# deepomicslab/PALACE

Measured on AMD Instinct MI355X. Metric: contigs/sec eref+generate_graph+matching, 1M-contig synth, 1/2/4/8 GPU, higher is better.
Workload: dtype u32

## Files before the change

palace_amd/csrc/decomp.hip:

```cpp
#include "decomp.hpp"

#include <algorithm>

namespace palace {

namespace {

constexpr uint64_t kNoKey = ~0ull;
constexpr uint64_t kClosed = 0;
constexpr int kStampShift = 42;
constexpr int kPackedShift = 52, kPackedStamps = 1 << (64 - kPackedShift);
constexpr uint64_t kLenMask = (1ull << 40) - 1;


__device__ __forceinline__ uint64_t wave_incl_scan(uint64_t v, int lane)
{
#pragma unroll
    for (int d = 1; d < 64; d <<= 1) {
        const uint64_t u = __shfl_up(v, d);
        if (lane >= d) v += u;
    }
    return v;
}

constexpr int kMaxWaves = 16;

__device__ void scan_partials_body(const uint64_t *__restrict__ in, int64_t n, uint64_t *__restrict__ partials, int blk, int nblk)
{
    __shared__ uint64_t part[kMaxWaves];
    const int64_t chunk = (n + nblk - 1) / nblk;
    const int64_t a = min(n, static_cast<int64_t>(blk) * chunk), e = min(n, a + chunk);
    uint64_t s = 0;
    for (int64_t i = a + threadIdx.x; i < e; i += blockDim.x) s += in[i];
    const int lane = threadIdx.x & 63, waves = static_cast<int>(blockDim.x >> 6);
    s = wave_incl_scan(s, lane);
    if (lane == 63) part[threadIdx.x >> 6] = s;
    __syncthreads();
    if (threadIdx.x == 0) {
        uint64_t t = 0;
        for (int w = 0; w < waves; w++) t += part[w];
        partials[blk] = t;
    }
    __syncthreads();
}

__device__ void scan_prefix_body(uint64_t *__restrict__ partials, int n_parts, uint64_t *__restrict__ total)
{
    __shared__ uint64_t part[kMaxWaves];
    const int lane = threadIdx.x & 63, wv = threadIdx.x >> 6;
    const uint64_t x = static_cast<int>(threadIdx.x) < n_parts ? partials[threadIdx.x] : 0;
    const uint64_t incl = wave_incl_scan(x, lane);
    if (lane == 63) part[wv] = incl;
    __syncthreads();
    uint64_t before = 0;
    for (int w = 0; w < wv; w++) before += part[w];
    if (static_cast<int>(threadIdx.x) < n_parts) partials[threadIdx.x] = before + incl - x;
    if (threadIdx.x == blockDim.x - 1) *total = before + incl;
    __syncthreads();
}

__device__ void scan_apply_body(const uint64_t *__restrict__ in, uint64_t *__restrict__ out, int64_t n, const uint64_t *__restrict__ partials,
                                int blk, int nblk)
{
    __shared__ uint64_t part[kMaxWaves];
    const int64_t chunk = (n + nblk - 1) / nblk;
    const int64_t a = min(n, static_cast<int64_t>(blk) * chunk), e = min(n, a + chunk);
    const int lane = threadIdx.x & 63, wv = threadIdx.x >> 6, waves = static_cast<int>(blockDim.x >> 6);
    uint64_t carry = partials[blk];
    for (int64_t base = a; base < e; base += blockDim.x) {
        const int64_t i = base + threadIdx.x;
        const uint64_t x = i < e ? in[i] : 0;
        const uint64_t incl = wave_incl_scan(x, lane);
        if (lane == 63) part[wv] = incl;
        __syncthreads();
        uint64_t before = 0, all = 0;
        for (int w = 0; w < waves; w++) { if (w < wv) before += part[w]; all += part[w]; }
        if (i < e) out[i] = carry + before + incl - x;
        carry += all;
        __syncthreads();
    }
}

__global__ __launch_bounds__(kDecompBlock) void scan_partials_kernel(const uint64_t *__restrict__ in, const int32_t *__restrict__ n_dev,
                                                                     uint64_t *__restrict__ partials)
{
    scan_partials_body(in, *n_dev, partials, static_cast<int>(blockIdx.x), static_cast<int>(gridDim.x));
}
__global__ __launch_bounds__(kDecompBlock) void scan_prefix_kernel(uint64_t *__restrict__ partials, int n_parts, uint64_t *__restrict__ total)
{
    scan_prefix_body(partials, n_parts, total);
}
__global__ __launch_bounds__(kDecompBlock) void scan_apply_kernel(const uint64_t *__restrict__ in, uint64_t *__restrict__ out,
                                                                  const int32_t *__restrict__ n_dev, const uint64_t *__restrict__ partials)
{
    scan_apply_body(in, out, *n_dev, partials, static_cast<int>(blockIdx.x), static_cast<int>(gridDim.x));
}

struct Span { int tid, n; };
__device__ __forceinline__ Span whole_grid() { return Span{static_cast<int>(blockIdx.x * blockDim.x + threadIdx.x), static_cast<int>(gridDim.x * blockDim.x)}; }

__device__ void ph_init(const DecompBufs &b, Span T, int64_t comp_cap, int64_t vert_cap, int n_flags, int allow_packed)
{
    DecompState *st = b.st;
    const int V = st->V;
    for (int i = T.tid; i < V; i += T.n) { b.bo_hi[i] = kNoKey; b.bi_hi[i] = kNoKey; b.on_path[i] = 0; }
    for (int i = T.tid; i < n_flags; i += T.n) b.changed[i] = 0;
    if (T.tid == 0) {
        st->n_comp = 0; st->n_vert = 0; st->comp_cap = comp_cap; st->vert_cap = vert_cap;
        st->unsettled = 0; st->overflow = 0; st->bad = 0; st->dead = 0; st->scan_total = 0; st->alive_after = 0;
        st->packed = (allow_packed && b.kc && b.pack_bad && *b.pack_bad == 0) ? 1u : 0u;
        if (comp_cap >= 0) b.o_off[0] = 0;
    }
}

__device__ void ph_round_begin(const DecompBufs &b, Span T, int reset_left)
{
    const int V = b.st->V;
    if (!reset_left && b.st->dead) return;
    if (T.tid == 0) { b.st->alive_after = 0; if (reset_left) b.st->dead = 0; }
    const int64_t E = b.st->E;
    for (int64_t e = T.tid; e < E; e += T.n) b.done[e] = 0;
    const bool packed = b.st->packed != 0;
    for (int i = T.tid; i < V; i += T.n) {
        const int s = i >> 1;
        const int64_t l = reset_left ? 1 : b.left[s];
        if (reset_left && !(i & 1)) b.left[s] = 1;
        b.alive[i] = l > 0;
        b.next[i] = -1; b.prev[i] = -1;
        b.bo_hi[i] = b.bi_hi[i] = l > 0 ? kNoKey : kClosed;
        if (!packed) { b.bo_lo[i] = kNoKey; b.bo_lo[V + i] = kNoKey; b.bi_lo[i] = kNoKey; b.bi_lo[V + i] = kNoKey; }
        b.len_a[i] = 0;
    }
}

struct IterArgs {
    uint64_t stamp;
    uint64_t stamp_p;
    int parity;
    int prev_flag, flag;
    int unique_hi;
};


__device__ void ph_propose_hi(const DecompBufs &b, Span T, const IterArgs &a)
{
    if (b.st->dead) return;
    if (a.prev_flag >= 0 && !b.changed[a.prev_flag]) return;
    const int64_t E = b.st->E;
    const int V = b.st->V;
    const int other = (a.parity ^ 1) * V;
    const bool packed = b.st->packed != 0;
    for (int64_t e = T.tid; e < E; e += T.n) {
        if (b.done[e]) continue;
        const int u = b.src[e], v = b.dst[e];
        if (b.bi_hi[v] == kClosed) { b.done[e] = 1; continue; }
        const uint64_t k = packed ? (a.stamp_p | b.kc[e]) : (a.stamp | b.khi[e]);
        if (atomicMin(reinterpret_cast<unsigned long long *>(&b.bo_hi[u]), static_cast<unsigned long long>(k)) == kClosed) { b.done[e] = 1; continue; }
        atomicMin(reinterpret_cast<unsigned long long *>(&b.bi_hi[v]), static_cast<unsigned long long>(k));
        if (!a.unique_hi && !packed) { b.bo_lo[other + u] = kNoKey; b.bi_lo[other + v] = kNoKey; }
    }
}

__device__ void ph_propose_lo(const DecompBufs &b, Span T, const IterArgs &a)
{
    if (b.st->dead) return;
    if (a.prev_flag >= 0 && !b.changed[a.prev_flag]) return;
    if (b.st->packed) return;
    const int64_t E = b.st->E;
    const int mine = a.parity * b.st->V;
    for (int64_t e = T.tid; e < E; e += T.n) {
        if (b.done[e]) continue;
        const int u = b.src[e], v = b.dst[e];
        const uint64_t k = a.stamp | b.khi[e], lo = b.klo[e];
        if (b.bo_hi[u] == k) atomicMin(reinterpret_cast<unsigned long long *>(&b.bo_lo[mine + u]), static_cast<unsigned long long>(lo));
        if (b.bi_hi[v] == k) atomicMin(reinterpret_cast<unsigned long long *>(&b.bi_lo[mine + v]), static_cast<unsigned long long>(lo));
    }
}

__device__ void ph_commit_flag(const DecompBufs &b, Span T, const IterArgs &a, volatile unsigned int *took);
__device__ void ph_commit(const DecompBufs &b, Span T, const IterArgs &a)
{
    if (b.st->dead) return;
    if (a.prev_flag >= 0 && !b.changed[a.prev_flag]) return;
    ph_commit_flag(b, T, a, b.changed + a.flag);
}
__device__ void ph_commit_flag(const DecompBufs &b, Span T, const IterArgs &a, volatile unsigned int *took)
{
    bool any = false;
    const int64_t E = b.st->E;
    const int mine = a.parity * b.st->V;
    const bool packed = b.st->packed != 0;
    for (int64_t e = T.tid; e < E; e += T.n) {
        if (b.done[e]) continue;
        const int u = b.src[e], v = b.dst[e];
        const uint64_t k = packed ? (a.stamp_p | b.kc[e]) : (a.stamp | b.khi[e]);
        if (b.bo_hi[u] != k || b.bi_hi[v] != k) continue;
        const uint64_t lo = b.klo[e];
        if (!a.unique_hi && !packed && (b.bo_lo[mine + u] != lo || b.bi_lo[mine + v] != lo)) continue;
        b.next[u] = v; b.prev[v] = u;
        b.nhi[u] = b.khi[e]; b.nlo[u] = lo;
        b.bo_hi[u] = kClosed; b.bi_hi[v] = kClosed;
        b.done[e] = 1;
        any = true;
    }
    if (__syncthreads_or(any) && threadIdx.x == 0) *took = 1u;
}

__device__ void ph_heads(const DecompBufs &b, Span T, int round, int last_flag)
{
    DecompState *st = b.st;
    if (st->dead) return;
    if (T.tid == 0 && last_flag >= 0 && b.changed[last_flag]) st->unsettled = 1;
    const int V = st->V;
    for (int v = T.tid; v < V; v += T.n) {
        if (!b.alive[v] || b.prev[v] >= 0) continue;
        int len = 0, last = v;
        int64_t least = b.left[v >> 1];
        for (int x = v; x >= 0; x = b.next[x]) {
            b.on_path[x] = round + 1;
            last = x;
            len++;
            least = min(least, b.left[x >> 1]);
        }
        const int twin_first = last ^ 1;
        if (v > twin_first) continue;
        const int64_t uses = twin_first == v ? 2 : 1;
        b.len_a[v] = (1ull << 40) | static_cast<uint64_t>(len);
        b.pay[v] = max(static_cast<int64_t>(1), least / uses);
        b.kind[v] = 0;
        b.open_at[v] = 0;
    }
}

__device__ void ph_cycles(const DecompBufs &b, Span T, int round)
{
    const int V = b.st->V;
    if (b.st->dead) return;
    for (int v = T.tid; v < V; v += T.n) {
        if (!b.alive[v] || b.on_path[v] == round + 1) continue;
        int len = 1, twin_least = v ^ 1, worst = 0;
        uint64_t whi = b.nhi[v], wlo = b.nlo[v];
        int64_t least = b.left[v >> 1];
        bool first = true;
        for (int x = b.next[v]; x != v; x = b.next[x]) {
            if (x < v) { first = false; break; }
            twin_least = min(twin_least, x ^ 1);
            const uint64_t hi = b.nhi[x], lo = b.nlo[x];
            if (hi > whi || (hi == whi && lo > wlo)) { whi = hi; wlo = lo; worst = len; }
            least = min(least, b.left[x >> 1]);
            len++;
        }
        if (!first || v > twin_least) continue;
        const int64_t uses = twin_least == v ? 2 : 1;
        b.len_a[v] = (1ull << 40) | static_cast<uint64_t>(len);
        b.pay[v] = max(static_cast<int64_t>(1), least / uses);
        b.kind[v] = 1;
        b.open_at[v] = (worst + 1) % len;
    }
}

__device__ void ph_emit(const DecompBufs &b, Span T, int round, int64_t c0, int64_t v0)
{
    DecompState *st = b.st;
    const int V = st->V;
    if (st->dead) return;
    int64_t alive = 0;
    for (int v = T.tid; v < V; v += T.n) {
        const uint64_t la = b.len_a[v];
        if (!la) continue;
        const int64_t len = static_cast<int64_t>(la & kLenMask);
        const uint64_t p = b.pos[v];
        const int64_t c = c0 + static_cast<int64_t>(p >> 40), at = v0 + static_cast<int64_t>(p & kLenMask);
        const int64_t pay = b.pay[v];
        const bool room = c < st->comp_cap && at + len <= st->vert_cap;
        if (!room) st->overflow = 1;
        else { b.o_off[c] = at; b.o_kind[c] = b.kind[v]; b.o_iter[c] = round; b.o_open[c] = b.open_at[v]; }
        int x = v;
        int64_t still = 0;
        for (int64_t k = 0; k < len; k++) {
            if (room) b.o_verts[at + k] = 2 * b.orig[x >> 1] + (x & 1);
            const int64_t l = b.left[x >> 1];
            b.left[x >> 1] = max(static_cast<int64_t>(0), l - pay);
            still += l - pay > 0;
            x = b.next[x];
        }
        alive += still;
    }
    __shared__ unsigned long long wg_alive;
    if (threadIdx.x == 0) wg_alive = 0;
    __syncthreads();
    if (alive) atomicAdd(&wg_alive, static_cast<unsigned long long>(alive));
    __syncthreads();
    if (threadIdx.x == 0 && wg_alive) atomicAdd(reinterpret_cast<unsigned long long *>(&st->alive_after), wg_alive);
}


__global__ void dec_init_kernel(DecompBufs b, int64_t comp_cap, int64_t vert_cap, int n_flags, int allow_packed) { ph_init(b, whole_grid(), comp_cap, vert_cap, n_flags, allow_packed); }
__global__ void dec_round_begin_kernel(DecompBufs b, int reset_left) { ph_round_begin(b, whole_grid(), reset_left); }
__global__ void dec_propose_hi_kernel(DecompBufs b, IterArgs a) { ph_propose_hi(b, whole_grid(), a); }
__global__ void dec_propose_lo_kernel(DecompBufs b, IterArgs a) { ph_propose_lo(b, whole_grid(), a); }
__global__ void dec_commit_kernel(DecompBufs b, IterArgs a) { ph_commit(b, whole_grid(), a); }
__global__ void dec_heads_kernel(DecompBufs b, int round, int last_flag) { ph_heads(b, whole_grid(), round, last_flag); }
__global__ void dec_cycles_kernel(DecompBufs b, int round) { ph_cycles(b, whole_grid(), round); }
__global__ void dec_emit_kernel(DecompBufs b, int round) { ph_emit(b, whole_grid(), round, b.st->n_comp, b.st->n_vert); }

__global__ void dec_round_end_kernel(DecompBufs b)
{
    DecompState *st = b.st;
    if (blockIdx.x || threadIdx.x || st->dead) return;
    st->dead = st->alive_after == 0;
    st->n_comp += static_cast<int64_t>(st->scan_total >> 40);
    st->n_vert += static_cast<int64_t>(st->scan_total & kLenMask);
    if (st->n_comp <= st->comp_cap) b.o_off[st->n_comp] = st->n_vert;
}

size_t up256(size_t v) { return (v + 255) / 256 * 256; }

struct Carver {
    char *base;
    size_t used = 0;
    template <class T>
    T *take(size_t n)
    {
        T *p = base ? reinterpret_cast<T *>(base + used) : nullptr;
        used += up256(std::max<size_t>(1, n) * sizeof(T));
        return p;
    }
};

size_t carve_all(DecompBufs &b, char *base, int64_t s_cap, int64_t e_cap, int64_t comp_cap, int64_t vert_cap, int rounds, int iters)
{
    Carver c{base};
    const size_t S = static_cast<size_t>(std::max<int64_t>(1, s_cap)), V = 2 * S, E = static_cast<size_t>(std::max<int64_t>(1, e_cap));
    b.st = c.take<DecompState>(1);
    b.src = c.take<int32_t>(E); b.dst = c.take<int32_t>(E);
    b.khi = c.take<uint64_t>(E); b.klo = c.take<uint64_t>(E);
    b.done = c.take<uint8_t>(E);
    b.kc = c.take<uint64_t>(E);
    b.left = c.take<int64_t>(S); b.orig = c.take<int32_t>(S);
    b.next = c.take<int32_t>(V); b.prev = c.take<int32_t>(V); b.on_path = c.take<int32_t>(V); b.open_at = c.take<int32_t>(V);
    b.nhi = c.take<uint64_t>(V); b.nlo = c.take<uint64_t>(V);
    b.bo_hi = c.take<uint64_t>(V); b.bi_hi = c.take<uint64_t>(V);
    b.bo_lo = c.take<uint64_t>(2 * V); b.bi_lo = c.take<uint64_t>(2 * V);
    b.len_a = c.take<uint64_t>(V); b.pos = c.take<uint64_t>(V);
    b.pay = c.take<int64_t>(V);
    b.alive = c.take<uint8_t>(V); b.kind = c.take<uint8_t>(V);
    b.partials = c.take<uint64_t>(kDecompGrid + 1);
    b.changed = c.take<uint32_t>(static_cast<size_t>(rounds) * static_cast<size_t>(iters));
    b.o_off = c.take<int64_t>(static_cast<size_t>(comp_cap) + 1);
    b.o_verts = c.take<int32_t>(static_cast<size_t>(vert_cap));
    b.o_iter = c.take<int32_t>(static_cast<size_t>(comp_cap));
    b.o_open = c.take<int32_t>(static_cast<size_t>(comp_cap));
    b.o_kind = c.take<uint8_t>(static_cast<size_t>(comp_cap));
    return c.used;
}

}

size_t decomp_bytes(int64_t s_cap, int64_t e_cap, int64_t comp_cap, int64_t vert_cap, int rounds, int iters)
{
    DecompBufs tmp;
    return carve_all(tmp, nullptr, s_cap, e_cap, comp_cap, vert_cap, rounds, iters);
}

void decomp_carve(DecompBufs &b, char *base, int64_t s_cap, int64_t e_cap, int64_t comp_cap, int64_t vert_cap, int rounds, int iters)
{
    carve_all(b, base, s_cap, e_cap, comp_cap, vert_cap, rounds, iters);
}

int scan_u64(palace_ctx *ctx, const uint64_t *in, uint64_t *out, const int32_t *n_dev, uint64_t *partials, uint64_t *total_dev)
{
    hipLaunchKernelGGL(scan_partials_kernel, dim3(kDecompGrid), dim3(kDecompBlock), 0, ctx->stream, in, n_dev, partials);
    hipLaunchKernelGGL(scan_prefix_kernel, dim3(1), dim3(kDecompBlock), 0, ctx->stream, partials, kDecompGrid, total_dev);
    hipLaunchKernelGGL(scan_apply_kernel, dim3(kDecompGrid), dim3(kDecompBlock), 0, ctx->stream, in, out, n_dev, partials);
    PALACE_HIP_TRY(hipGetLastError());
    return PALACE_OK;
}

namespace {

const dim3 kBlock(kDecompBlock);
constexpr int kWideGridDefault = 2048;
inline dim3 wide_grid(const palace_ctx *ctx) { return dim3(ctx->match_grid > 0 ? ctx->match_grid : kWideGridDefault); }

void enqueue_iterations(palace_ctx *ctx, const DecompBufs &b, int first, int n, uint64_t *count, int flag0, bool unique_hi)
{
    for (int k = 0; k < n; k++) {
        IterArgs a{((1ull << 21) - 1 - *count) << kStampShift, static_cast<uint64_t>((kPackedStamps - 1 - *count) & (kPackedStamps - 1)) << kPackedShift,
                   (first + k) & 1, k ? flag0 + k - 1 : -1, flag0 + k, unique_hi ? 1 : 0};
        (*count)++;
        hipLaunchKernelGGL(dec_propose_hi_kernel, wide_grid(ctx), kBlock, 0, ctx->stream, b, a);
        if (!unique_hi) hipLaunchKernelGGL(dec_propose_lo_kernel, wide_grid(ctx), kBlock, 0, ctx->stream, b, a);
        hipLaunchKernelGGL(dec_commit_kernel, wide_grid(ctx), kBlock, 0, ctx->stream, b, a);
    }
}

int enqueue_read_off(palace_ctx *ctx, const DecompBufs &b, int round, int last_flag)
{
    hipLaunchKernelGGL(dec_heads_kernel, wide_grid(ctx), kBlock, 0, ctx->stream, b, round, last_flag);
    hipLaunchKernelGGL(dec_cycles_kernel, wide_grid(ctx), kBlock, 0, ctx->stream, b, round);
    int rc = scan_u64(ctx, b.len_a, b.pos, &b.st->V, b.partials, &b.st->scan_total);
    if (rc) return rc;
    hipLaunchKernelGGL(dec_emit_kernel, wide_grid(ctx), kBlock, 0, ctx->stream, b, round);
    hipLaunchKernelGGL(dec_round_end_kernel, dim3(1), dim3(64), 0, ctx->stream, b);
    PALACE_HIP_TRY(hipGetLastError());
    return PALACE_OK;
}

}

int decomp_begin(palace_ctx *ctx, const DecompBufs &b, int rounds, int64_t comp_cap, int64_t vert_cap)
{
    PALACE_REQUIRE(rounds >= 1 && rounds <= kMaxRounds, "round count out of range");
    static_assert(kDecompGrid <= kDecompBlock, "scan_prefix_kernel scans the block sums with one workgroup");
    const int allow_packed = !ctx->match_two_word_keys && static_cast<int64_t>(rounds) * kMaxIters < kPackedStamps ? 1 : 0;
    hipLaunchKernelGGL(dec_init_kernel, wide_grid(ctx), kBlock, 0, ctx->stream, b, comp_cap, vert_cap, rounds * kMaxIters, allow_packed);
    PALACE_HIP_TRY(hipGetLastError());
    return PALACE_OK;
}

int decomp_rounds(palace_ctx *ctx, const DecompBufs &b, int t0, int t1, int rounds, int aggressive, int iters, bool unique_hi,
                  uint64_t *count)
{
    PALACE_REQUIRE(0 <= t0 && t0 <= t1 && t1 <= rounds && rounds <= kMaxRounds && iters >= 1 && iters <= kMaxIters, "round / iteration count out of range");
    for (int t = t0; t < t1; t++) {
        hipLaunchKernelGGL(dec_round_begin_kernel, wide_grid(ctx), kBlock, 0, ctx->stream, b, (aggressive && t == rounds - 1) ? 1 : 0);
        enqueue_iterations(ctx, b, 0, iters, count, t * kMaxIters, unique_hi);
        int rc = enqueue_read_off(ctx, b, t, t * kMaxIters + iters - 1);
        if (rc) return rc;
    }
    PALACE_HIP_TRY(hipGetLastError());
    return PALACE_OK;
}

int decomp_run_checked(palace_ctx *ctx, const DecompBufs &b, int rounds, int aggressive, bool unique_hi, int64_t comp_cap,
                       int64_t vert_cap, int64_t max_iterations, uint64_t *iterations_out)
{
    PALACE_REQUIRE(rounds >= 1 && rounds <= kMaxRounds, "round count out of range");
    constexpr int kBatch = 16;
    hipLaunchKernelGGL(dec_init_kernel, wide_grid(ctx), kBlock, 0, ctx->stream, b, comp_cap, vert_cap, kBatch, 0);
    uint64_t count = 0;
    for (int t = 0; t < rounds; t++) {
        hipLaunchKernelGGL(dec_round_begin_kernel, wide_grid(ctx), kBlock, 0, ctx->stream, b, (aggressive && t == rounds - 1) ? 1 : 0);
        for (int first = 0;; first += kBatch) {
            PALACE_HIP_TRY(hipMemsetAsync(b.changed, 0, kBatch * sizeof(uint32_t), ctx->stream));
            enqueue_iterations(ctx, b, first, kBatch, &count, 0, unique_hi);
            uint32_t last = 0;
            PALACE_HIP_TRY(hipMemcpyAsync(&last, b.changed + kBatch - 1, sizeof last, hipMemcpyDeviceToHost, ctx->stream));
            PALACE_HIP_TRY(hipStreamSynchronize(ctx->stream));
            if (!last) break;
            if (static_cast<int64_t>(count) > max_iterations || count + kBatch >= (1ull << 21)) {
                set_error("matching: no fixed point after %llu iterations", static_cast<unsigned long long>(count));
                return PALACE_ESTATE;
            }
        }
        PALACE_HIP_TRY(hipMemsetAsync(b.changed, 0, kBatch * sizeof(uint32_t), ctx->stream));
        int rc = enqueue_read_off(ctx, b, t, kBatch - 1);
        if (rc) return rc;
    }
    if (iterations_out) *iterations_out = count;
    return PALACE_OK;
}

int decomp_group(palace_ctx *ctx, const DecompBufs &b, DecompRun &run, int rounds, int aggressive, bool unique_hi)
{
    const int first = kFirstGroupRounds;
    const int t0 = run.next_round, t1 = std::min(rounds, t0 + (t0 == 0 ? first : kRoundsPerGroup));
    for (int t = t0; t < t1; t++) {
        const int iters = ctx->match_iters > 0 ? std::min(ctx->match_iters, kMaxIters) : (t == 0 ? kFirstRoundIters : kLaterRoundIters);
        int rc = decomp_rounds(ctx, b, t, t + 1, rounds, aggressive, iters, unique_hi, &run.count);
        if (rc) return rc;
        run.rounds++;
    }
    run.next_round = t1;
    return PALACE_OK;
}

int decomp_finish(palace_ctx *ctx, const DecompBufs &b, DecompRun &run, int rounds, int aggressive, bool unique_hi, int64_t comp_cap,
                  int64_t vert_cap, int64_t max_iterations, DecompState *h_state, const std::function<int()> &reset_left)
{
    for (;;) {
        PALACE_HIP_TRY(hipMemcpyAsync(h_state, b.st, sizeof *h_state, hipMemcpyDeviceToHost, ctx->stream));
        PALACE_HIP_TRY(hipStreamSynchronize(ctx->stream));
        if (h_state->unsettled) {
            int rc = reset_left();
            if (rc) return rc;
            run.checked = true; run.rounds = rounds; run.count = 0;
            rc = decomp_run_checked(ctx, b, rounds, aggressive, unique_hi, comp_cap, vert_cap, max_iterations, &run.count);
            if (rc) return rc;
            PALACE_HIP_TRY(hipMemcpyAsync(h_state, b.st, sizeof *h_state, hipMemcpyDeviceToHost, ctx->stream));
            PALACE_HIP_TRY(hipStreamSynchronize(ctx->stream));
            return PALACE_OK;
        }
        if (run.next_round >= rounds) return PALACE_OK;
        if (h_state->alive_after == 0) {
            if (!aggressive) return PALACE_OK;
            run.next_round = rounds - 1;
        }
        int rc = decomp_group(ctx, b, run, rounds, aggressive, unique_hi);
        if (rc) return rc;
    }
}

}
```

palace_amd/csrc/decomp.hpp:

```cpp
#pragma once
#include <functional>

#include "common.hpp"

struct palace_match_result {
    int64_t n = 0;
    int64_t *off = nullptr;
    int32_t *verts = nullptr, *iter = nullptr, *open_at = nullptr;
    uint8_t *kind = nullptr;
    uint64_t *bare = nullptr;
    int64_t n_bare = 0;
    bool borrowed = false;
    ~palace_match_result();
};

namespace palace {

constexpr int kDecompGrid = 256;
constexpr int kDecompBlock = 256;
constexpr int kMaxRounds = 1024;
constexpr int kMaxIters = 64;

struct DecompState {
    int32_t S, V;
    int64_t E;
    int64_t n_comp, n_vert;
    int64_t comp_cap, vert_cap;
    uint32_t unsettled;
    uint32_t overflow;
    uint32_t bad;
    uint32_t dead;
    uint32_t packed;
    uint64_t scan_total;
    int64_t alive_after;
};

struct DecompBufs {
    DecompState *st = nullptr;
    int32_t *src = nullptr, *dst = nullptr;
    uint64_t *khi = nullptr, *klo = nullptr;
    uint8_t *done = nullptr;
    uint64_t *kc = nullptr;
    const uint32_t *pack_bad = nullptr;
    int64_t *left = nullptr;
    int32_t *orig = nullptr;
    int32_t *next = nullptr, *prev = nullptr, *on_path = nullptr, *open_at = nullptr;
    uint64_t *nhi = nullptr, *nlo = nullptr;
    uint64_t *bo_hi = nullptr, *bi_hi = nullptr;
    uint64_t *bo_lo = nullptr, *bi_lo = nullptr;
    uint64_t *len_a = nullptr, *pos = nullptr;
    int64_t *pay = nullptr;
    uint8_t *alive = nullptr, *kind = nullptr;
    uint64_t *partials = nullptr;
    uint32_t *changed = nullptr;
    int64_t *o_off = nullptr;
    int32_t *o_verts = nullptr, *o_iter = nullptr, *o_open = nullptr;
    uint8_t *o_kind = nullptr;
};

size_t decomp_bytes(int64_t s_cap, int64_t e_cap, int64_t comp_cap, int64_t vert_cap, int rounds, int iters);
void decomp_carve(DecompBufs &b, char *base, int64_t s_cap, int64_t e_cap, int64_t comp_cap, int64_t vert_cap, int rounds, int iters);
constexpr int kFirstRoundIters = 7, kLaterRoundIters = 4, kRoundsPerGroup = 5, kFirstGroupRounds = 5;
int decomp_begin(palace_ctx *ctx, const DecompBufs &b, int rounds, int64_t comp_cap, int64_t vert_cap);
int decomp_rounds(palace_ctx *ctx, const DecompBufs &b, int t0, int t1, int rounds, int aggressive, int iters, bool unique_hi,
                  uint64_t *count);

struct DecompRun { int next_round = 0; uint64_t count = 0; int rounds = 0; bool checked = false; };
int decomp_group(palace_ctx *ctx, const DecompBufs &b, DecompRun &run, int rounds, int aggressive, bool unique_hi);
int decomp_finish(palace_ctx *ctx, const DecompBufs &b, DecompRun &run, int rounds, int aggressive, bool unique_hi, int64_t comp_cap,
                  int64_t vert_cap, int64_t max_iterations, DecompState *h_state, const std::function<int()> &reset_left);

int decomp_run_checked(palace_ctx *ctx, const DecompBufs &b, int rounds, int aggressive, bool unique_hi, int64_t comp_cap,
                       int64_t vert_cap, int64_t max_iterations, uint64_t *iterations_out = nullptr);

inline void decomp_note_run(palace_ctx *ctx, const DecompRun &run, const DecompState &h_state, bool unique_hi)
{
    ctx->match_last[0] = unique_hi ? 0 : (h_state.packed ? 2 : 1);
    ctx->match_last[1] = run.checked ? 1 : 0;
    ctx->match_last[2] = run.rounds;
    ctx->match_last[3] = static_cast<int64_t>(run.count);
}

int scan_u64(palace_ctx *ctx, const uint64_t *in, uint64_t *out, const int32_t *n_dev, uint64_t *partials, uint64_t *total_dev);

}
```

Before: 112.7 million.

## Replace edge-parallel atomicMin matching with per-vertex compacted adjacency lists

Builds per-vertex out/in adjacency lists once at decomposition start (count, scan, fill) and rewrites each matching iteration as a per-slot scan that drops closed neighbours, compacts the list in place and picks the best arc, with long lists handled by a whole wave. Commit becomes vertex-parallel, checking that both endpoints chose the same arc. This removes the per-iteration pass over all edges with 64-bit atomicMin, the separate lo-key propose kernel, and the stamp bookkeeping. In exchange it adds list-building kernels, more memory for entries, and irregular per-vertex work that may be imbalanced.

```diff
diff --git a/palace_amd/csrc/decomp.hip b/palace_amd/csrc/decomp.hip
--- a/palace_amd/csrc/decomp.hip
+++ b/palace_amd/csrc/decomp.hip
@@ -6,10 +6,8 @@
 
 namespace {
 
-constexpr uint64_t kNoKey = ~0ull;
-constexpr uint64_t kClosed = 0;
-constexpr int kStampShift = 42;
-constexpr int kPackedShift = 52, kPackedStamps = 1 << (64 - kPackedShift);
+constexpr int kPackedStamps = 1 << 12;
+constexpr int kLongList = 64;
 constexpr uint64_t kLenMask = (1ull << 40) - 1;
 
 
@@ -103,13 +101,38 @@
 {
     DecompState *st = b.st;
     const int V = st->V;
-    for (int i = T.tid; i < V; i += T.n) { b.bo_hi[i] = kNoKey; b.bi_hi[i] = kNoKey; b.on_path[i] = 0; }
+    for (int i = T.tid; i < V; i += T.n) { b.cnt[i] = 0; b.cnt[V + i] = 0; b.on_path[i] = 0; }
     for (int i = T.tid; i < n_flags; i += T.n) b.changed[i] = 0;
     if (T.tid == 0) {
         st->n_comp = 0; st->n_vert = 0; st->comp_cap = comp_cap; st->vert_cap = vert_cap;
-        st->unsettled = 0; st->overflow = 0; st->bad = 0; st->dead = 0; st->scan_total = 0; st->alive_after = 0;
+        st->unsettled = 0; st->overflow = 0; st->slots = 2 * V; st->dead = 0; st->scan_total = 0; st->alive_after = 0;
         st->packed = (allow_packed && b.kc && b.pack_bad && *b.pack_bad == 0) ? 1u : 0u;
         if (comp_cap >= 0) b.o_off[0] = 0;
+    }
+}
+
+__device__ void ph_list_count(const DecompBufs &b, Span T)
+{
+    const int64_t E = b.st->E;
+    const int V = b.st->V;
+    for (int64_t e = T.tid; e < E; e += T.n) {
+        b.place[2 * e] = atomicAdd(reinterpret_cast<int *>(&b.cnt[b.src[e]]), 1);
+        b.place[2 * e + 1] = atomicAdd(reinterpret_cast<int *>(&b.cnt[V + b.dst[e]]), 1);
+    }
+}
+
+__device__ void ph_list_fill(const DecompBufs &b, Span T)
+{
+    const int64_t E = b.st->E;
+    const int V = b.st->V;
+    const bool packed = b.st->packed != 0;
+    for (int64_t e = T.tid; e < E; e += T.n) {
+        const int u = b.src[e], v = b.dst[e];
+        const uint64_t k0 = packed ? b.kc[e] : b.khi[e];
+        const uint64_t out = b.off[u] + static_cast<uint64_t>(b.place[2 * e]), in = b.off[V + v] + static_cast<uint64_t>(b.place[2 * e + 1]);
+        b.ent[out] = ListEntry{static_cast<int32_t>(e), v, k0};
+        b.ent[in] = ListEntry{static_cast<int32_t>(e), u, k0};
+        if (!packed) { const uint64_t k1 = b.klo[e]; b.ent_k1[out] = k1; b.ent_k1[in] = k1; }
     }
 }
 
@@ -118,92 +141,166 @@
     const int V = b.st->V;
     if (!reset_left && b.st->dead) return;
     if (T.tid == 0) { b.st->alive_after = 0; if (reset_left) b.st->dead = 0; }
-    const int64_t E = b.st->E;
-    for (int64_t e = T.tid; e < E; e += T.n) b.done[e] = 0;
-    const bool packed = b.st->packed != 0;
     for (int i = T.tid; i < V; i += T.n) {
         const int s = i >> 1;
         const int64_t l = reset_left ? 1 : b.left[s];
         if (reset_left && !(i & 1)) b.left[s] = 1;
         b.alive[i] = l > 0;
         b.next[i] = -1; b.prev[i] = -1;
-        b.bo_hi[i] = b.bi_hi[i] = l > 0 ? kNoKey : kClosed;
-        if (!packed) { b.bo_lo[i] = kNoKey; b.bo_lo[V + i] = kNoKey; b.bi_lo[i] = kNoKey; b.bi_lo[V + i] = kNoKey; }
+        b.open[i] = b.open[V + i] = l > 0;
+        b.head[i] = SlotHead{b.off[i], l > 0 ? static_cast<int32_t>(b.cnt[i]) : 0, -1};
+        b.head[V + i] = SlotHead{b.off[V + i], l > 0 ? static_cast<int32_t>(b.cnt[V + i]) : 0, -1};
         b.len_a[i] = 0;
     }
 }
 
 struct IterArgs {
-    uint64_t stamp;
-    uint64_t stamp_p;
-    int parity;
     int prev_flag, flag;
     int unique_hi;
 };
 
 
-__device__ void ph_propose_hi(const DecompBufs &b, Span T, const IterArgs &a)
+struct Best { int32_t arc; uint64_t k0, k1; };
+__device__ __forceinline__ void take_better(Best &m, int32_t arc, uint64_t k0, uint64_t k1)
+{
+    if (arc >= 0 && (m.arc < 0 || k0 < m.k0 || (k0 == m.k0 && k1 < m.k1))) m = Best{arc, k0, k1};
+}
+
+__device__ void list_by_thread(const DecompBufs &b, int s, int flip, const SlotHead &h, bool two)
+{
+    constexpr int kAhead = 4;
+    ListEntry *L = b.ent + h.off;
+    uint64_t *K1 = b.ent_k1 + h.off;
+    const int n = h.live;
+    Best m{-1, 0, 0};
+    int w = 0;
+    for (int i0 = 0; i0 < n; i0 += kAhead) {
+        ListEntry x[kAhead];
+        uint64_t x1[kAhead];
+        bool keep[kAhead];
+#pragma unroll
+        for (int k = 0; k < kAhead; k++) {
+            x[k] = L[min(i0 + k, n - 1)];
+            x1[k] = two ? K1[min(i0 + k, n - 1)] : 0;
+        }
+#pragma unroll
+        for (int k = 0; k < kAhead; k++) keep[k] = i0 + k < n && b.open[flip + x[k].other] != 0;
+#pragma unroll
+        for (int k = 0; k < kAhead; k++) {
+            if (!keep[k]) continue;
+            take_better(m, x[k].arc, x[k].key, x1[k]);
+            if (w != i0 + k) {
+                L[i0 + k] = L[w]; L[w] = x[k];
+                if (two) { K1[i0 + k] = K1[w]; K1[w] = x1[k]; }
+            }
+            w++;
+        }
+    }
+    b.head[s].live = w;
+    b.head[s].best = m.arc;
+}
+
+__device__ __forceinline__ void loads_done()
+{
+    asm volatile("s_waitcnt vmcnt(0)" ::: "memory");
+}
+__device__ void list_by_wave(const DecompBufs &b, int s, int flip, bool two, int lane)
+{
+    const SlotHead h = b.head[s];
+    ListEntry *L = b.ent + h.off;
+    uint64_t *K1 = b.ent_k1 + h.off;
+    const int n = h.live;
+    const uint64_t below = (1ull << lane) - 1;
+    Best m{-1, 0, 0};
+    int w = 0;
+    for (int r = 0; r < n; r += 64) {
+        const int tn = min(64, n - r), d = r - w;
+        const bool have = lane < tn;
+        ListEntry x;
+        x.arc = -1; x.other = 0; x.key = 0;
+        uint64_t x1 = 0;
+        bool keep = false;
+        if (have) {
+            x = L[r + lane];
+            if (two) x1 = K1[r + lane];
+            keep = b.open[flip + x.other] != 0;
+        }
+        const uint64_t km = __ballot(keep), dm = __ballot(have && !keep);
+        const int c = __popcll(km), rk = __popcll(km & below), rd = __popcll(dm & below);
+        if (keep) take_better(m, x.arc, x.key, x1);
+        if (c && (d || dm)) {
+            if (d < 64) {
+                ListEntry y = x;
+                uint64_t y1 = 0;
+                if (lane < d) { y = L[w + lane]; if (two) y1 = K1[w + lane]; }
+                loads_done();
+                if (keep) { L[w + rk] = x; if (two) K1[w + rk] = x1; }
+                if (lane < d) { L[w + c + lane] = y; if (two) K1[w + c + lane] = y1; }
+                if (have && !keep) { L[w + c + d + rd] = x; if (two) K1[w + c + d + rd] = x1; }
+            } else {
+                ListEntry y = x;
+                uint64_t y1 = 0;
+                if (keep) { y = L[w + rk]; if (two) y1 = K1[w + rk]; }
+                loads_done();
+                if (keep) {
+                    L[w + rk] = x; L[r + lane] = y;
+                    if (two) { K1[w + rk] = x1; K1[r + lane] = y1; }
+                }
+            }
+        }
+        w += c;
+    }
+#pragma unroll
+    for (int d = 32; d; d >>= 1) {
+        const int32_t arc = __shfl_xor(m.arc, d);
+        const uint64_t k0 = __shfl_xor(m.k0, d), k1 = __shfl_xor(m.k1, d);
+        take_better(m, arc, k0, k1);
+    }
+    if (lane == 0) { b.head[s].live = w; b.head[s].best = m.arc; }
+}
+
+__device__ void ph_propose(const DecompBufs &b, const IterArgs &a)
 {
     if (b.st->dead) return;
     if (a.prev_flag >= 0 && !b.changed[a.prev_flag]) return;
-    const int64_t E = b.st->E;
-    const int V = b.st->V;
-    const int other = (a.parity ^ 1) * V;
-    const bool packed = b.st->packed != 0;
-    for (int64_t e = T.tid; e < E; e += T.n) {
-        if (b.done[e]) continue;
-        const int u = b.src[e], v = b.dst[e];
-        if (b.bi_hi[v] == kClosed) { b.done[e] = 1; continue; }
-        const uint64_t k = packed ? (a.stamp_p | b.kc[e]) : (a.stamp | b.khi[e]);
-        if (atomicMin(reinterpret_cast<unsigned long long *>(&b.bo_hi[u]), static_cast<unsigned long long>(k)) == kClosed) { b.done[e] = 1; continue; }
-        atomicMin(reinterpret_cast<unsigned long long *>(&b.bi_hi[v]), static_cast<unsigned long long>(k));
-        if (!a.unique_hi && !packed) { b.bo_lo[other + u] = kNoKey; b.bi_lo[other + v] = kNoKey; }
-    }
-}
-
-__device__ void ph_propose_lo(const DecompBufs &b, Span T, const IterArgs &a)
+    const int V = b.st->V, n_slots = 2 * V;
+    const bool two = !a.unique_hi && !b.st->packed;
+    const int lane = static_cast<int>(threadIdx.x & 63);
+    const int64_t step = static_cast<int64_t>(gridDim.x) * blockDim.x;
+    for (int64_t base = (static_cast<int64_t>(blockIdx.x) * blockDim.x + threadIdx.x) & ~63ll; base < n_slots; base += step) {
+        const int s = static_cast<int>(base) + lane;
+        bool is_long = false;
+        if (s < n_slots) {
+            const SlotHead h = b.head[s];
+            if (h.live > kLongList) is_long = true;
+            else if (h.live > 0) list_by_thread(b, s, s < V ? V : 0, h, two);
+        }
+        for (uint64_t todo = __ballot(is_long); todo; todo &= todo - 1) {
+            const int t = static_cast<int>(base) + __ffsll(static_cast<unsigned long long>(todo)) - 1;
+            list_by_wave(b, t, t < V ? V : 0, two, lane);
+        }
+    }
+}
+
+__device__ void ph_commit(const DecompBufs &b, Span T, const IterArgs &a)
 {
     if (b.st->dead) return;
     if (a.prev_flag >= 0 && !b.changed[a.prev_flag]) return;
-    if (b.st->packed) return;
-    const int64_t E = b.st->E;
-    const int mine = a.parity * b.st->V;
-    for (int64_t e = T.tid; e < E; e += T.n) {
-        if (b.done[e]) continue;
-        const int u = b.src[e], v = b.dst[e];
-        const uint64_t k = a.stamp | b.khi[e], lo = b.klo[e];
-        if (b.bo_hi[u] == k) atomicMin(reinterpret_cast<unsigned long long *>(&b.bo_lo[mine + u]), static_cast<unsigned long long>(lo));
-        if (b.bi_hi[v] == k) atomicMin(reinterpret_cast<unsigned long long *>(&b.bi_lo[mine + v]), static_cast<unsigned long long>(lo));
-    }
-}
-
-__device__ void ph_commit_flag(const DecompBufs &b, Span T, const IterArgs &a, volatile unsigned int *took);
-__device__ void ph_commit(const DecompBufs &b, Span T, const IterArgs &a)
-{
-    if (b.st->dead) return;
-    if (a.prev_flag >= 0 && !b.changed[a.prev_flag]) return;
-    ph_commit_flag(b, T, a, b.changed + a.flag);
-}
-__device__ void ph_commit_flag(const DecompBufs &b, Span T, const IterArgs &a, volatile unsigned int *took)
-{
     bool any = false;
-    const int64_t E = b.st->E;
-    const int mine = a.parity * b.st->V;
-    const bool packed = b.st->packed != 0;
-    for (int64_t e = T.tid; e < E; e += T.n) {
-        if (b.done[e]) continue;
-        const int u = b.src[e], v = b.dst[e];
-        const uint64_t k = packed ? (a.stamp_p | b.kc[e]) : (a.stamp | b.khi[e]);
-        if (b.bo_hi[u] != k || b.bi_hi[v] != k) continue;
-        const uint64_t lo = b.klo[e];
-        if (!a.unique_hi && !packed && (b.bo_lo[mine + u] != lo || b.bi_lo[mine + v] != lo)) continue;
+    const int V = b.st->V;
+    for (int u = T.tid; u < V; u += T.n) {
+        const SlotHead h = b.head[u];
+        const int32_t e = h.best;
+        if (h.live <= 0 || e < 0) continue;
+        const int v = b.dst[e];
+        if (b.head[V + v].best != e) continue;
         b.next[u] = v; b.prev[v] = u;
-        b.nhi[u] = b.khi[e]; b.nlo[u] = lo;
-        b.bo_hi[u] = kClosed; b.bi_hi[v] = kClosed;
-        b.done[e] = 1;
+        b.nhi[u] = b.khi[e]; b.nlo[u] = b.klo[e];
+        b.open[u] = 0; b.open[V + v] = 0;
+        b.head[u].live = 0; b.head[V + v].live = 0;
         any = true;
     }
-    if (__syncthreads_or(any) && threadIdx.x == 0) *took = 1u;
+    if (__syncthreads_or(any) && threadIdx.x == 0) b.changed[a.flag] = 1u;
 }
 
 __device__ void ph_heads(const DecompBufs &b, Span T, int round, int last_flag)
@@ -297,8 +394,9 @@
 
 __global__ void dec_init_kernel(DecompBufs b, int64_t comp_cap, int64_t vert_cap, int n_flags, int allow_packed) { ph_init(b, whole_grid(), comp_cap, vert_cap, n_flags, allow_packed); }
 __global__ void dec_round_begin_kernel(DecompBufs b, int reset_left) { ph_round_begin(b, whole_grid(), reset_left); }
-__global__ void dec_propose_hi_kernel(DecompBufs b, IterArgs a) { ph_propose_hi(b, whole_grid(), a); }
-__global__ void dec_propose_lo_kernel(DecompBufs b, IterArgs a) { ph_propose_lo(b, whole_grid(), a); }
+__global__ void dec_list_count_kernel(DecompBufs b) { ph_list_count(b, whole_grid()); }
+__global__ void dec_list_fill_kernel(DecompBufs b) { ph_list_fill(b, whole_grid()); }
+__global__ __launch_bounds__(kDecompBlock) void dec_propose_kernel(DecompBufs b, IterArgs a) { ph_propose(b, a); }
 __global__ void dec_commit_kernel(DecompBufs b, IterArgs a) { ph_commit(b, whole_grid(), a); }
 __global__ void dec_heads_kernel(DecompBufs b, int round, int last_flag) { ph_heads(b, whole_grid(), round, last_flag); }
 __global__ void dec_cycles_kernel(DecompBufs b, int round) { ph_cycles(b, whole_grid(), round); }
@@ -335,13 +433,13 @@
     b.st = c.take<DecompState>(1);
     b.src = c.take<int32_t>(E); b.dst = c.take<int32_t>(E);
     b.khi = c.take<uint64_t>(E); b.klo = c.take<uint64_t>(E);
-    b.done = c.take<uint8_t>(E);
     b.kc = c.take<uint64_t>(E);
+    b.ent = c.take<ListEntry>(2 * E); b.ent_k1 = c.take<uint64_t>(2 * E); b.place = c.take<int32_t>(2 * E);
     b.left = c.take<int64_t>(S); b.orig = c.take<int32_t>(S);
     b.next = c.take<int32_t>(V); b.prev = c.take<int32_t>(V); b.on_path = c.take<int32_t>(V); b.open_at = c.take<int32_t>(V);
     b.nhi = c.take<uint64_t>(V); b.nlo = c.take<uint64_t>(V);
-    b.bo_hi = c.take<uint64_t>(V); b.bi_hi = c.take<uint64_t>(V);
-    b.bo_lo = c.take<uint64_t>(2 * V); b.bi_lo = c.take<uint64_t>(2 * V);
+    b.cnt = c.take<uint64_t>(2 * V); b.off = c.take<uint64_t>(2 * V);
+    b.head = c.take<SlotHead>(2 * V); b.open = c.take<uint8_t>(2 * V);
     b.len_a = c.take<uint64_t>(V); b.pos = c.take<uint64_t>(V);
     b.pay = c.take<int64_t>(V);
     b.alive = c.take<uint8_t>(V); b.kind = c.take<uint8_t>(V);
@@ -383,16 +481,25 @@
 constexpr int kWideGridDefault = 2048;
 inline dim3 wide_grid(const palace_ctx *ctx) { return dim3(ctx->match_grid > 0 ? ctx->match_grid : kWideGridDefault); }
 
-void enqueue_iterations(palace_ctx *ctx, const DecompBufs &b, int first, int n, uint64_t *count, int flag0, bool unique_hi)
+void enqueue_iterations(palace_ctx *ctx, const DecompBufs &b, int n, uint64_t *count, int flag0, bool unique_hi)
 {
     for (int k = 0; k < n; k++) {
-        IterArgs a{((1ull << 21) - 1 - *count) << kStampShift, static_cast<uint64_t>((kPackedStamps - 1 - *count) & (kPackedStamps - 1)) << kPackedShift,
-                   (first + k) & 1, k ? flag0 + k - 1 : -1, flag0 + k, unique_hi ? 1 : 0};
+        IterArgs a{k ? flag0 + k - 1 : -1, flag0 + k, unique_hi ? 1 : 0};
         (*count)++;
-        hipLaunchKernelGGL(dec_propose_hi_kernel, wide_grid(ctx), kBlock, 0, ctx->stream, b, a);
-        if (!unique_hi) hipLaunchKernelGGL(dec_propose_lo_kernel, wide_grid(ctx), kBlock, 0, ctx->stream, b, a);
+        hipLaunchKernelGGL(dec_propose_kernel, wide_grid(ctx), kBlock, 0, ctx->stream, b, a);
         hipLaunchKernelGGL(dec_commit_kernel, wide_grid(ctx), kBlock, 0, ctx->stream, b, a);
     }
+}
+
+int enqueue_begin(palace_ctx *ctx, const DecompBufs &b, int64_t comp_cap, int64_t vert_cap, int n_flags, int allow_packed)
+{
+    hipLaunchKernelGGL(dec_init_kernel, wide_grid(ctx), kBlock, 0, ctx->stream, b, comp_cap, vert_cap, n_flags, allow_packed);
+    hipLaunchKernelGGL(dec_list_count_kernel, wide_grid(ctx), kBlock, 0, ctx->stream, b);
+    int rc = scan_u64(ctx, b.cnt, b.off, &b.st->slots, b.partials, &b.st->scan_total);
+    if (rc) return rc;
+    hipLaunchKernelGGL(dec_list_fill_kernel, wide_grid(ctx), kBlock, 0, ctx->stream, b);
+    PALACE_HIP_TRY(hipGetLastError());
+    return PALACE_OK;
 }
 
 int enqueue_read_off(palace_ctx *ctx, const DecompBufs &b, int round, int last_flag)
@@ -414,9 +521,7 @@
     PALACE_REQUIRE(rounds >= 1 && rounds <= kMaxRounds, "round count out of range");
     static_assert(kDecompGrid <= kDecompBlock, "scan_prefix_kernel scans the block sums with one workgroup");
     const int allow_packed = !ctx->match_two_word_keys && static_cast<int64_t>(rounds) * kMaxIters < kPackedStamps ? 1 : 0;
-    hipLaunchKernelGGL(dec_init_kernel, wide_grid(ctx), kBlock, 0, ctx->stream, b, comp_cap, vert_cap, rounds * kMaxIters, allow_packed);
-    PALACE_HIP_TRY(hipGetLastError());
-    return PALACE_OK;
+    return enqueue_begin(ctx, b, comp_cap, vert_cap, rounds * kMaxIters, allow_packed);
 }
 
 int decomp_rounds(palace_ctx *ctx, const DecompBufs &b, int t0, int t1, int rounds, int aggressive, int iters, bool unique_hi,
@@ -425,7 +530,7 @@
     PALACE_REQUIRE(0 <= t0 && t0 <= t1 && t1 <= rounds && rounds <= kMaxRounds && iters >= 1 && iters <= kMaxIters, "round / iteration count out of range");
     for (int t = t0; t < t1; t++) {
         hipLaunchKernelGGL(dec_round_begin_kernel, wide_grid(ctx), kBlock, 0, ctx->stream, b, (aggressive && t == rounds - 1) ? 1 : 0);
-        enqueue_iterations(ctx, b, 0, iters, count, t * kMaxIters, unique_hi);
+        enqueue_iterations(ctx, b, iters, count, t * kMaxIters, unique_hi);
         int rc = enqueue_read_off(ctx, b, t, t * kMaxIters + iters - 1);
         if (rc) return rc;
     }
@@ -438,24 +543,25 @@
 {
     PALACE_REQUIRE(rounds >= 1 && rounds <= kMaxRounds, "round count out of range");
     constexpr int kBatch = 16;
-    hipLaunchKernelGGL(dec_init_kernel, wide_grid(ctx), kBlock, 0, ctx->stream, b, comp_cap, vert_cap, kBatch, 0);
+    int rc = enqueue_begin(ctx, b, comp_cap, vert_cap, kBatch, 0);
+    if (rc) return rc;
     uint64_t count = 0;
     for (int t = 0; t < rounds; t++) {
         hipLaunchKernelGGL(dec_round_begin_kernel, wide_grid(ctx), kBlock, 0, ctx->stream, b, (aggressive && t == rounds - 1) ? 1 : 0);
-        for (int first = 0;; first += kBatch) {
+        for (;;) {
             PALACE_HIP_TRY(hipMemsetAsync(b.changed, 0, kBatch * sizeof(uint32_t), ctx->stream));
-            enqueue_iterations(ctx, b, first, kBatch, &count, 0, unique_hi);
+            enqueue_iterations(ctx, b, kBatch, &count, 0, unique_hi);
             uint32_t last = 0;
             PALACE_HIP_TRY(hipMemcpyAsync(&last, b.changed + kBatch - 1, sizeof last, hipMemcpyDeviceToHost, ctx->stream));
             PALACE_HIP_TRY(hipStreamSynchronize(ctx->stream));
             if (!last) break;
-            if (static_cast<int64_t>(count) > max_iterations || count + kBatch >= (1ull << 21)) {
+            if (static_cast<int64_t>(count) > max_iterations) {
                 set_error("matching: no fixed point after %llu iterations", static_cast<unsigned long long>(count));
                 return PALACE_ESTATE;
             }
         }
         PALACE_HIP_TRY(hipMemsetAsync(b.changed, 0, kBatch * sizeof(uint32_t), ctx->stream));
-        int rc = enqueue_read_off(ctx, b, t, kBatch - 1);
+        rc = enqueue_read_off(ctx, b, t, kBatch - 1);
         if (rc) return rc;
     }
     if (iterations_out) *iterations_out = count;
diff --git a/palace_amd/csrc/decomp.hpp b/palace_amd/csrc/decomp.hpp
--- a/palace_amd/csrc/decomp.hpp
+++ b/palace_amd/csrc/decomp.hpp
@@ -28,26 +28,33 @@
     int64_t comp_cap, vert_cap;
     uint32_t unsettled;
     uint32_t overflow;
-    uint32_t bad;
+    int32_t slots;
     uint32_t dead;
     uint32_t packed;
     uint64_t scan_total;
     int64_t alive_after;
 };
 
+struct alignas(16) ListEntry { int32_t arc, other; uint64_t key; };
+
+struct alignas(16) SlotHead { uint64_t off; int32_t live, best; };
+
 struct DecompBufs {
     DecompState *st = nullptr;
     int32_t *src = nullptr, *dst = nullptr;
     uint64_t *khi = nullptr, *klo = nullptr;
-    uint8_t *done = nullptr;
     uint64_t *kc = nullptr;
     const uint32_t *pack_bad = nullptr;
     int64_t *left = nullptr;
     int32_t *orig = nullptr;
     int32_t *next = nullptr, *prev = nullptr, *on_path = nullptr, *open_at = nullptr;
     uint64_t *nhi = nullptr, *nlo = nullptr;
-    uint64_t *bo_hi = nullptr, *bi_hi = nullptr;
-    uint64_t *bo_lo = nullptr, *bi_lo = nullptr;
+    ListEntry *ent = nullptr;
+    uint64_t *ent_k1 = nullptr;
+    int32_t *place = nullptr;
+    uint64_t *cnt = nullptr, *off = nullptr;
+    SlotHead *head = nullptr;
+    uint8_t *open = nullptr;
     uint64_t *len_a = nullptr, *pos = nullptr;
     int64_t *pay = nullptr;
     uint8_t *alive = nullptr, *kind = nullptr;
```

Measured after the change: 113.0 million, median of 2. No clear change (+0.2%).
